# lukefleed/two-pass-lanczos

Hardware: AMD Instinct MI355X
Metric: Lanczos iterations/sec + SpMV GB/s (vs HBM roofline), 500k-arc KKT k=500 (higher is better)
Workload: dtype f64

## Files before the change

two-pass-lanczos_amd/csrc/tpl_device.h:

```cpp
#pragma once
#include <stdint.h>

namespace tpl {

constexpr int kTPB = 256;
#ifndef TPL_CHUNK_ROWS
#define TPL_CHUNK_ROWS 512
#endif
constexpr int kChunkRows = TPL_CHUNK_ROWS;
constexpr int kRowsPerThread = kChunkRows / kTPB;
#ifndef TPL_ELEM_ROWS
#define TPL_ELEM_ROWS 2048
#endif
constexpr int kElemRows = TPL_ELEM_ROWS;
constexpr int kElemMinBlocks = 192;
constexpr int kShortRowMax = 32;
#ifndef TPL_MAX_SLICES
#define TPL_MAX_SLICES 8
#endif
constexpr int kSlices = TPL_MAX_SLICES;
#ifndef TPL_SLOT_STRIDE
#define TPL_SLOT_STRIDE TPL_MAX_SLICES
#endif
constexpr int kSlotStride = TPL_SLOT_STRIDE;
// ... 15 lines not shown
constexpr int kWinLoads = kWinMax / 256;
constexpr int kFusedWidth = 4;
constexpr int kFusedHubMax = kTPB;
constexpr int kFusedLongMax = 2048;
constexpr int kBinMax = 7936;
constexpr int kCntStride = 16;
constexpr double kBreakdownTol = 2.220446049250313080847263336181640625e-13;

inline int p2_flush(int j, int last) {
  return (j % 3 == 0 || j == last) ? j - ((j - 1) / 3) * 3 : 0;
}

struct BinSeg {
  int32_t start, ri, row, pad;
};

struct CsrDev {
  const int32_t* srows;
  const void* s_col;
  const int32_t* s_cbase;
  const void* s_val;
  const int32_t* c_base;
  const int32_t* c_width;
  const void* b_col;
  const int32_t* b_cbase;
  const void* b_val;
  const BinSeg* b_seg;
  const int32_t* b_hdr;
  double* P;
  unsigned int* Pcnt;
// ... 128 lines not shown
```

two-pass-lanczos_amd/csrc/tpl_k_p2_fused.hip:

```cpp
#include "tpl_klaunch.h"

namespace tpl {

constexpr int kHubAhead = 8;

struct FusedP2Args {
  const int32_t* h_row;
  const int32_t* h_ent;
  const double* h_val;
  int32_t n_open, n_hub;
  double* ycache;
  const double* rec;
  const int32_t* flags;
  const double* v1;
  double* x;
  int64_t n;
  int32_t n_long;
  int32_t steps;
  const void* s_col;
  const void* s_val;
  const int32_t* s_cbase;
  const int32_t* c_base;
  const int32_t* c_width;
  int32_t n_short, n_chunks, s_width, val_i8, s_col16;
};

// ... 9 lines not shown
  return {readlane_f64(cv, 0), readlane_f64(cv, 1), readlane_f64(cv, 2), readlane_f64(cv, 3)};
}
__device__ __forceinline__ void fused_step_r(double s, const StepRec& r, double& vc, double& vp,
                                             double& xv) {
  double w = s - r.beta_sub * vp;
  w = w - r.alpha * vc;
  const double vn = w * r.invb;
  xv = xv + r.ycoef * vn;
  vp = vc;
  vc = vn;
}
__device__ __forceinline__ void fused_step(double s, double cv, double& vc, double& vp, double& xv) {
  fused_step_r(s, rec_fields(cv), vc, vp, xv);
}

constexpr uint32_t kLaneOff = 0x80000000u;
__device__ __forceinline__ void st_cache_row(double* row, int nl, uint32_t off, double v) {
  typedef uint32_t u32x2 __attribute__((ext_vector_type(2)));
  const __amdgpu_buffer_rsrc_t r = __builtin_amdgcn_make_buffer_rsrc(row, 0, nl * 8, 0x00020000);
  u32x2 d;
  d.x = (uint32_t)__double2loint(v);
  d.y = (uint32_t)__double2hiint(v);
  __builtin_amdgcn_raw_buffer_store_b64(d, r, off, 0, 0);
}

enum HubMode { kHubLong, kHubLds, kHubWave };
constexpr int kWave = 64;
template <HubMode MODE>
__device__ __forceinline__ void hub_chain(const FusedP2Args& a, double (*vh)[kTPB], int last,
                                          int lc, bool writes, bool open,
                                          const int (&ent)[kFusedWidth],
                                          const double (&av)[kFusedWidth], double& vc, double& vp,
                                          double& xv) {
  const int t = threadIdx.x;
  const int nl = a.n_long;
  double yb[kHubAhead], cb[kHubAhead];
#pragma unroll
  for (int u = 0; u < kHubAhead; ++u) {
    const int jj = clampi(1 + u, last);
    yb[u] = a.ycache[(size_t)(jj - 1) * nl + lc];
    cb[u] = a.rec[8 * (size_t)jj + (t & 7)];
  }
  const uint32_t soff = writes ? (uint32_t)lc * 8u : kLaneOff;
  auto step = [&](int j, double s, double cv) {
    st_cache_row(a.ycache + (size_t)(j - 1) * nl, nl, soff, vc);
    if (MODE == kHubLds) {
      double* vb = vh[j & 1];
      vb[t] = vc;
      __syncthreads();
      if (open) {
        s = 0.0;
#pragma unroll
        for (int k = 0; k < kFusedWidth; ++k) {
          const double prod = av[k] * vb[ent[k] < 0 ? 0 : ent[k]];
          s = s + (ent[k] >= 0 ? prod : -0.0);
        }
      }
    }
    if (MODE == kHubWave) {
      double so = 0.0;
#pragma unroll
      for (int k = 0; k < kFusedWidth; ++k) {
        const double prod = av[k] * __shfl(vc, ent[k] < 0 ? 0 : ent[k], kWave);
        so = so + (ent[k] >= 0 ? prod : -0.0);
      }
      s = open ? so : s;
    }
    fused_step(s, cv, vc, vp, xv);
  };
  const int nblk = last / kHubAhead;
  int j0 = 1;
  if (nblk > 0) __builtin_amdgcn_s_waitcnt(0x0F70);
  for (int b = 0; b < nblk; ++b, j0 += kHubAhead) {
#pragma unroll
    for (int u = 0; u < kHubAhead; ++u) {
      const int j = j0 + u;
      step(j, yb[u], cb[u]);
      __builtin_amdgcn_sched_barrier(0);
      const int jn = clampi(j + kHubAhead, last);
      yb[u] = a.ycache[(size_t)(jn - 1) * nl + lc];
      cb[u] = a.rec[8 * (size_t)jn + (t & 7)];
    }
  }
  const int rem = last - nblk * kHubAhead;
#pragma unroll
  for (int u = 0; u < kHubAhead - 1; ++u) {
    if (u >= rem) break;
    step(j0 + u, yb[u], cb[u]);
  }
}

__global__ __launch_bounds__(kTPB) void k_p2_hub(FusedP2Args a) {
  __shared__ double vh[2][kTPB];
  const int steps = fused_steps(a);
  if (steps < 2) return;
  const int last = steps - 1;
  const int t = threadIdx.x;
  const int nl = a.n_long;
  const int64_t first_long = a.n - nl;
  const int n_lb = (nl + kTPB - 1) / kTPB;
  const bool hub = (int)blockIdx.x >= n_lb;
  bool live, open = false;
  int lc;
  int64_t row;
  int ent[kFusedWidth];
  double av[kFusedWidth];
#pragma unroll
  for (int k = 0; k < kFusedWidth; ++k) {
    ent[k] = -1;
    av[k] = 0.0;
  }
  if (hub) {
    live = t < a.n_hub;
    open = t < a.n_open;
    row = a.h_row[clampi(t, a.n_hub - 1)];
    lc = open ? 0 : clampi((int)(row - first_long), nl - 1);
    if (open) {
#pragma unroll
      for (int k = 0; k < kFusedWidth; ++k) {
        ent[k] = a.h_ent[t * kFusedWidth + k];
        av[k] = a.h_val[t * kFusedWidth + k];
      }
    }
  } else {
    const int l = blockIdx.x * kTPB + t;
    lc = clampi(l, nl - 1);
    row = first_long + lc;
    live = l < nl;
    for (int h = a.n_open; h < a.n_hub; ++h) live = live && a.h_row[h] != (int32_t)row;
  }
  double vc = a.v1[row], vp = 0.0, xv = a.x[row];
  if (hub && a.n_hub <= kWave) {
    if (t >= kWave) return;
    hub_chain<kHubWave>(a, vh, last, lc, live && !open, open, ent, av, vc, vp, xv);
  } else if (hub) {
    hub_chain<kHubLds>(a, vh, last, lc, live && !open, open, ent, av, vc, vp, xv);
  } else {
    hub_chain<kHubLong>(a, vh, last, lc, live, false, ent, av, vc, vp, xv);
  }
  if (live) st_out(a.x + row, xv);
}

__device__ __forceinline__ int fused_col(const FusedP2Args& a, int e, int cbase) {
  if (a.s_col16) {
    const int off = reinterpret_cast<const uint16_t*>(a.s_col)[e];
    return off == 0xFFFF ? -1 : cbase + off;
  }
  return reinterpret_cast<const int32_t*>(a.s_col)[e];
}
__device__ __forceinline__ double fused_val(const FusedP2Args& a, int e) {
  if (a.val_i8) return (double)reinterpret_cast<const int8_t*>(a.s_val)[e];
  return reinterpret_cast<const double*>(a.s_val)[e];
}

constexpr int kRowsGroup = 4;
constexpr int kRowsThreads = kTPB * kRowsGroup;
constexpr int kRowsDepth = 2;

template <int W, int NL>
__global__ __launch_bounds__(kRowsThreads) void k_p2_rows(FusedP2Args a) {
  extern __shared__ double lds[];
  constexpr int NLC = (NL + kRowsGroup - 1) / kRowsGroup;
  constexpr int D = kRowsDepth;
  const int steps = fused_steps(a);
  if (steps < 2) return;
  const int last = steps - 1;
  const int tw = threadIdx.x;
  const int t = tw % kTPB;
  const int chunk_w = blockIdx.x * kRowsGroup + tw / kTPB;
  const bool have = chunk_w < a.n_chunks;
  const int chunk = have ? chunk_w : a.n_chunks - 1;
  const int nl = a.n_long;
  const int first_long = (int)(a.n - nl);
  const int wc = a.s_width > 0 ? a.s_width : a.c_width[chunk];
  const int base = a.s_width > 0 ? chunk * kChunkRows * a.s_width : a.c_base[chunk];
  const bool packed = a.s_width > 0 && packed_chunk_width(a.s_width);
  const int cbase = a.s_col16 ? a.s_cbase[chunk] : 0;
  int row[kRowsPerThread];
  bool live[kRowsPerThread];
  int li[kRowsPerThread][W];
  double av[kRowsPerThread][W];
// ... 20 lines not shown
      li[q][k] = idx;
    }
    vc[q] = a.v1[row[q]];
    vp[q] = 0.0;
    xv[q] = a.x[row[q]];
  }
  double st[D][NLC], cvr[D];
#pragma unroll
  for (int d = 0; d < D; ++d) {
    const int jj = clampi(1 + d, last);
#pragma unroll
    for (int u = 0; u < NLC; ++u)
      st[d][u] = a.ycache[(size_t)(jj - 1) * nl + clampi(tw + u * kRowsThreads, nl - 1)];
    cvr[d] = a.rec[8 * (size_t)jj + (tw & 7)];
  }
  auto step = [&](int j, int d, auto refill) {
    double* vb = lds + (j & 1) * nl;
#pragma unroll
    for (int u = 0; u < NLC; ++u)
      if (u < NLC - 1 || tw + u * kRowsThreads < nl) vb[tw + u * kRowsThreads] = st[d][u];
    const StepRec r = rec_fields(cvr[d]);
    if (decltype(refill)::value) {
      __builtin_amdgcn_sched_barrier(0);
      const int jn = clampi(j + D, last);
#pragma unroll
      for (int u = 0; u < NLC; ++u)
        st[d][u] = a.ycache[(size_t)(jn - 1) * nl + clampi(tw + u * kRowsThreads, nl - 1)];
      cvr[d] = a.rec[8 * (size_t)jn + (tw & 7)];
    }
    __syncthreads();
#pragma unroll
    for (int q = 0; q < kRowsPerThread; ++q) {
      double s = 0.0;
#pragma unroll
      for (int k = 0; k < W; ++k) {
        const double g = vb[li[q][k] < 0 ? 0 : li[q][k]];
        const double prod = av[q][k] * (li[q][k] == -2 ? vc[q] : g);
        s = s + (li[q][k] != -1 ? prod : -0.0);
      }
      fused_step_r(s, r, vc[q], vp[q], xv[q]);
    }
  };
  const int nblk = last / D;
  int j0 = 1;
  if (nblk > 0) __builtin_amdgcn_s_waitcnt(0x0F70);
  for (int b = 0; b < nblk; ++b, j0 += D) {
#pragma unroll
    for (int d = 0; d < D; ++d) step(j0 + d, d, std::true_type{});
  }
  const int rem = last - nblk * D;
#pragma unroll
  for (int d = 0; d < D - 1; ++d) {
    if (d >= rem) break;
    step(j0 + d, d, std::false_type{});
  }
#pragma unroll
  for (int q = 0; q < kRowsPerThread; ++q)
    if (live[q]) st_out(a.x + row[q], xv[q]);
}

namespace launch {

static FusedP2Args fused_args(const CsrDev& A, const DevState& S, const double* ycache,
                              const double* v1, double* x, int steps) {
  FusedP2Args a{};
  a.ycache = const_cast<double*>(ycache);
  a.rec = S.p2c;
  a.flags = S.flags;
  a.v1 = v1;
  a.x = x;
  a.n = A.n;
  a.n_long = A.n_long;
  a.steps = steps;
  a.s_col = A.s_col;
  a.s_val = A.s_val;
  a.s_cbase = A.s_cbase;
  a.c_base = A.c_base;
  a.c_width = A.c_width;
  a.n_short = A.n_short;
  a.n_chunks = A.n_chunks;
  a.s_width = A.s_width;
  a.val_i8 = A.val_i8;
  a.s_col16 = A.s_col16;
  return a;
}

hipError_t p2_fused_hub(const CsrDev& A, const DevState& S, const FusedP2Dev& H, double* ycache,
                        const double* v1, double* x, int steps, hipStream_t s) {
  if (A.n_long <= 0 || !A.s_identity || H.n_hub > kFusedHubMax || H.n_open > H.n_hub)
    return hipErrorInvalidConfiguration;
  FusedP2Args a = fused_args(A, S, ycache, v1, x, steps);
  a.h_row = H.h_row;
  a.h_ent = H.h_ent;
  a.h_val = H.h_val;
  a.n_open = H.n_open;
  a.n_hub = H.n_hub;
  const int grid = (A.n_long + kTPB - 1) / kTPB + (H.n_hub > 0 ? 1 : 0);
  hipLaunchKernelGGL(k_p2_hub, dim3(grid), dim3(kTPB), 0, s, a);
  return hipGetLastError();
}

template <int W, int... NLs>
static bool rows_nl(int nloads, const FusedP2Args& a, int grid, size_t lds, hipStream_t s,
                    std::integer_sequence<int, NLs...>) {
  auto one = [&](auto NL) {
    if (nloads != decltype(NL)::value + 1) return false;
    hipLaunchKernelGGL((k_p2_rows<W, decltype(NL)::value + 1>), dim3(grid), dim3(kRowsThreads),
                       lds, s, a);
    return true;
  };
  return (one(std::integral_constant<int, NLs>{}) || ...);
}

hipError_t p2_fused_rows(const CsrDev& A, const DevState& S, const double* ycache,
                         const double* v1, double* x, int steps, hipStream_t s) {
  if (A.n_long <= 0 || A.n_long > kFusedLongMax || !A.s_identity)
    return hipErrorInvalidConfiguration;
  if (A.n_chunks <= 0) return hipSuccess;
  const FusedP2Args a = fused_args(A, S, ycache, v1, x, steps);
  const size_t lds = 2 * (size_t)A.n_long * sizeof(double);
  const int nloads = (A.n_long + kTPB - 1) / kTPB;
  constexpr auto nls = std::make_integer_sequence<int, kFusedLongMax / kTPB>{};
  const int w = A.s_width > 0 ? A.s_width : kFusedWidth;
  const int grid = (A.n_chunks + kRowsGroup - 1) / kRowsGroup;
  bool ok = false;
  switch (w) {
    case 1: ok = rows_nl<1>(nloads, a, grid, lds, s, nls); break;
    case 2: ok = rows_nl<2>(nloads, a, grid, lds, s, nls); break;
    case 3: ok = rows_nl<3>(nloads, a, grid, lds, s, nls); break;
    case 4: ok = rows_nl<4>(nloads, a, grid, lds, s, nls); break;
    default: break;
  }
  return ok ? hipGetLastError() : hipErrorInvalidConfiguration;
}

}
}
```

two-pass-lanczos_amd/csrc/tpl_kcommon.h:

```cpp
#pragma once
#include <hip/hip_runtime.h>
#include "tpl_device.h"
#include "tpl_lab.h"

namespace tpl {

template <int kCtrl>
__device__ __forceinline__ double dpp_f64(double v) {
  const long long b = __double_as_longlong(v);
  const int lo = __builtin_amdgcn_update_dpp(0, (int)b, kCtrl, 0xF, 0xF, false);
  const int hi = __builtin_amdgcn_update_dpp(0, (int)(b >> 32), kCtrl, 0xF, 0xF, false);
  return __longlong_as_double(((long long)hi << 32) | (unsigned int)lo);
}
__device__ __forceinline__ double swz_xor16_f64(double v) {
  const long long b = __double_as_longlong(v);
  const int lo = __builtin_amdgcn_ds_swizzle((int)b, 0x401F);
  const int hi = __builtin_amdgcn_ds_swizzle((int)(b >> 32), 0x401F);
  return __longlong_as_double(((long long)hi << 32) | (unsigned int)lo);
}
__device__ __forceinline__ double readlane_f64(double v, int l) {
  const long long b = __double_as_longlong(v);
  const int lo = __builtin_amdgcn_readlane((int)b, l);
  const int hi = __builtin_amdgcn_readlane((int)(b >> 32), l);
  return __longlong_as_double(((long long)hi << 32) | (unsigned int)lo);
// ... 84 lines not shown

struct PreNone {};
__device__ __forceinline__ bool defer_long_y(const CsrDev& A, int ri, double y) {
  if (!A.long_defer) return false;
  A.ypart[ri] = y;
  return true;
}
struct EpiSpmv {
  double* y;
  __device__ __forceinline__ PreNone pre(int) const { return {}; }
  __device__ __forceinline__ double apply(int i, double s, const PreNone&, double&) const {
    st_out(y + i, s);
    return s;
  }
  __device__ __forceinline__ void long_alpha(int, double) const {}
  __device__ __forceinline__ bool long_y(const CsrDev& A, int ri, double y) const {
    return defer_long_y(A, ri, y);
  }
};

struct Pre1 {
  double rc, rp;
};
struct EpiPass1 {
  const double* r_cur;
  const double* r_prev;
  bool has_prev;
  double invN_cur, invN_prev, beta_sub;
  double* W;
  double* Vcol;
  double* Pa_long;
  __device__ __forceinline__ Pre1 pre(int i) const { return Pre1{r_cur[i], r_prev[i]}; }
  __device__ __forceinline__ void long_alpha(int r, double acc) const { st_out(Pa_long + r, acc); }
  __device__ __forceinline__ bool long_y(const CsrDev& A, int ri, double y) const {
    double* yp = A.ypart;
    if (yp) st_out(yp + ri, y);
    return A.long_defer != 0;
  }
  __device__ __forceinline__ double apply(int i, double s, const Pre1& p, double& acc) const {
    const double v = p.rc * invN_cur;
    const double vp = has_prev ? p.rp * invN_prev : 0.0;
    const double w = s - beta_sub * vp;
    st_out(W + i, w);
    if (Vcol) Vcol[i] = v;
    acc = fma(v, w, acc);
    return v;
  }
};

struct Pre2R {
  double vc, vp, x, cv;
};
// ... 30 lines not shown
    const double vp = has_prev ? p.vp : 0.0;
    double w = s - beta_sub * vp;
    w = w - alpha * p.vc;
    const double vn = w * invb;
    st_out(v_next + i, vn);
    if (nflush) {
      double xv = p.x;
      if (nflush >= 3) xv = xv + readlane_f64(p.cv, 5) * p.vp;
      if (nflush >= 2) xv = xv + readlane_f64(p.cv, 4) * p.vc;
      st_out(x + i, xv + ycoef * vn);
    }
    if (Vcol) Vcol[i] = vn;
    return vn;
  }
  __device__ __forceinline__ void long_alpha(int, double) const {}
  __device__ __forceinline__ bool long_y(const CsrDev& A, int ri, double y) const {
    return defer_long_y(A, ri, y);
  }
};

__device__ __forceinline__ void pin_layout_args(const CsrDev& A) {
  asm volatile("" ::"s"(A.s_col), "s"(A.s_val), "s"(A.s_cbase), "s"(A.b_col), "s"(A.b_val),
               "s"(A.b_seg), "s"(A.b_hdr), "s"(A.b_cbase));
  asm volatile("" ::"s"(A.n_short), "s"(A.n_slice_blocks), "s"(A.n_slices), "s"(A.bin_cap),
               "s"(A.s_identity), "s"(A.n_chunks));
}

__device__ __forceinline__ void keep_pre(PreNone&) {}
__device__ __forceinline__ void keep_pre(Pre1& p) { keep(p.rc); keep(p.rp); }
__device__ __forceinline__ void keep_pre(Pre2R& p) { keep(p.vc); keep(p.vp); keep(p.x); keep(p.cv); }

// ... 322 lines not shown
        acc = group8_sum(acc);
        if (g8 == 0 && valid) psum[j] = acc;
      }
    }
  }
  TPL_MARK(7);
  TPL_MARK(8);
  __syncthreads();
  TPL_MARK(3);
  keep_pre(pre);
  if (sg.ri < 0) return;
  const double p = psum[t];
  const int ns = A.n_slices;
  if (ns == 1 || sg.pad == 0) {
    const double y = 0.0 + p;
    if (epi.long_y(A, sg.ri, y)) return;
    double acc = 0.0;
    epi.apply(sg.row, y, pre, acc);
    epi.long_alpha(sg.ri, acc);
    return;
  }
  unsigned long long* slots = reinterpret_cast<unsigned long long*>(A.P + (size_t)sg.ri * kSlotStride);
  __hip_atomic_store(slots + s, (unsigned long long)__double_as_longlong(p), __ATOMIC_RELAXED,
                     __HIP_MEMORY_SCOPE_AGENT);
  asm volatile("s_waitcnt vmcnt(0)" ::: "memory");
  TPL_MARK(4);
  const unsigned int arrived = __builtin_amdgcn_atomic_inc32(
      A.Pcnt + (size_t)sg.ri * kCntStride, (unsigned)sg.pad, __ATOMIC_RELAXED, "agent");
  asm volatile("" ::: "memory");
  if (arrived != (unsigned)sg.pad) return;
  static_assert(kSlices == 8, "four slot pairs");
// ... 7 lines not shown
  asm volatile(
      "global_load_dwordx4 %0, %4, off sc1\n\t"
      "global_load_dwordx4 %1, %5, off sc1\n\t"
      "global_load_dwordx4 %2, %6, off sc1\n\t"
      "global_load_dwordx4 %3, %7, off sc1\n\t"
      "s_waitcnt vmcnt(0)"
      : "=&v"(r0), "=&v"(r1), "=&v"(r2), "=&v"(r3)
      : "v"(p0), "v"(p1), "v"(p2), "v"(p3)
      : "memory");
  v[0] = r0.x; v[1] = r0.y; v[2] = r1.x; v[3] = r1.y;
  v[4] = r2.x; v[5] = r2.y; v[6] = r3.x; v[7] = r3.y;
  double y = 0.0;
#pragma unroll
  for (int k = 0; k < kSlices; ++k)
    if (k < ns) y = y + __longlong_as_double((long long)v[k]);
  if (epi.long_y(A, sg.ri, y)) return;
  double acc = 0.0;
  epi.apply(sg.row, y, pre, acc);
  epi.long_alpha(sg.ri, acc);
}

__device__ __forceinline__ int rb_first(int G2, int x) { return (x * G2 + 7) >> 3; }
__device__ __forceinline__ int elem_block(int G2, int i) {
  const int x = i & 7, q = i >> 3;
  const int rb = rb_first(G2, x) + q;
  return rb < rb_first(G2, x + 1) ? rb : -1;
}
__device__ __forceinline__ int elem_block(const CsrDev& A, int i) { return elem_block(A.G2, i); }
__device__ __forceinline__ int chunk_of_block(const CsrDev& A, int i) {
  const int cpe = (int)(A.E / kChunkRows);
  const int x = (i + A.n_slice_blocks) & 7, q = i >> 3;
// ... 162 lines not shown
```

two-pass-lanczos_amd/csrc/tpl_launch.h:

```cpp
#pragma once
#include <hip/hip_runtime.h>

#include "tpl_device.h"

namespace tpl {
struct BatchDev;
namespace launch {
hipError_t spmv(const CsrDev& A, const double* x, double* y, hipStream_t s);
hipError_t p1_init(const CsrDev& A, const DevState& S, const double* b, hipStream_t s);
hipError_t p1_spmv(const CsrDev& A, const DevState& S, const double* xsrc, const double* r_cur,
                   const double* r_prev, double* W, double* Vcol, int j, hipStream_t s,
                   unsigned long long* stamp = nullptr);
hipError_t p1_axpy(const CsrDev& A, const DevState& S, const double* W, const double* r_cur,
                   double* r_next, int j, int k, int elim, hipStream_t s,
                   unsigned long long* stamp = nullptr);
hipError_t p1_axpy_tol(const CsrDev& A, const DevState& S, const double* W, const double* r_cur,
                       double* r_next, int j, int k, double* tr, hipStream_t s);
hipError_t p1_tol_fin(const DevState& S, double* tr, hipStream_t s);
struct ShiftTol {
  const double* tol;
  const double* sig;
  double* lu;
  double* st;
  double* res;
// ... 20 lines not shown
                               double* Y, int32_t* back, int scale, hipStream_t s);
hipError_t p2_init(int64_t n, const DevState& S, const double* b, double* v1, double* x,
                   double* Vcol, int dyn, hipStream_t s);
hipError_t p2_spmv(const CsrDev& A, const DevState& S, const double* xsrc, const double* v_cur,
                   const double* v_prev, double* v_next, double* x, double* Vcol, int j,
                   int nflush, hipStream_t s);
hipError_t p2_cached(const CsrDev& A, const DevState& S, const double* xsrc, const double* v_cur,
                     const double* v_prev, double* v_next, double* x, double* Vcol,
                     const double* ycache, const int32_t* lrow, int j, int nflush,
                     hipStream_t s);
struct FusedP2Dev {
  const int32_t *h_row, *h_ent;
  const double* h_val;
  int32_t n_open, n_hub;
};
hipError_t p2_fused_hub(const CsrDev& A, const DevState& S, const FusedP2Dev& H, double* ycache,
                        const double* v1, double* x, int steps, hipStream_t s);
hipError_t p2_fused_rows(const CsrDev& A, const DevState& S, const double* ycache,
                         const double* v1, double* x, int steps, hipStream_t s);
hipError_t bp2_cached(int nb, const CsrDev& A, const BatchDev& B, const double* v_cur,
                      const double* v_prev, double* v_next, double* x, const double* ycrow,
                      const int32_t* lrow, int j, hipStream_t s);
hipError_t p2_coefs(const DevState& S, int k, int dyn, hipStream_t s);
hipError_t gemv_recon(int64_t n, int steps, const DevState& S, const double* V, double* x,
                      hipStream_t s);
hipError_t p2_minit(const CsrDev& A, const DevState& S, const double* Y, int ldy, const double* b,
                    double* v1, double* X, int64_t ldx, int m, hipStream_t s);
hipError_t p2_xacc(const CsrDev& A, const double* Y, int ldy, int j, int nflush, const double* vp,
                   const double* vc, const double* vn, double* X, int64_t ldx, int m,
                   hipStream_t s);
int long_epi_blocks(const CsrDev& A);
hipError_t long_epi_p1(const CsrDev& A, const DevState& S, const double* yall, int R,
                       const double* r_cur, const double* r_prev, double* W, double* Vcol,
                       double* Pa_long, int j, hipStream_t s);
// ... 14 lines not shown
```

two-pass-lanczos_amd/csrc/tpl_op.h:

```cpp
#pragma once
#include <hip/hip_runtime.h>

#include <algorithm>
#include <cstdlib>
#include <cstring>
#include <functional>
#include <map>
#include <memory>
#include <new>
#include <string>
#include <vector>

#include "tpl_batch.h"
#include "tpl_device.h"
#include "tpl_internal.h"
#include "tpl_launch.h"
#include "tpl_layout.h"
#include "tpl_partition.h"

typedef struct ncclComm* ncclComm_t;

namespace tpl {

#define HIPCHK(expr)                                                                        \
// ... 227 lines not shown

struct HostDecomp {
  int32_t flags[kFlagBytes / 4];
  double b_norm;
  const double* alphas;
  const double* betas;
  size_t steps;
};

bool use_graphs();
GraphExec capture_graph(tpl_op_s* op, const std::function<void()>& enqueue);
void enqueue_reorth(tpl_op_s* op, int j, int mode);
void enqueue_p1_prologue(tpl_op_s* op);
void enqueue_p1_step(tpl_op_s* op, int j, int k, double* Vcol, bool elim = false,
                     unsigned long long* st1 = nullptr, unsigned long long* st2 = nullptr,
                     double* ycrow = nullptr);
void launch_p2_step(tpl_op_s* op, const CsrDev& A, int j, int t, int nflush, double* Vcol);
void launch_bp2_step(tpl_op_s* op, const CsrDev& A, int nb, int j);
void enqueue_pass2(tpl_op_s* op, size_t steps, double* Vout);
void enqueue_ftk_only(tpl_op_s* op, size_t k, int f, int scale);
void run_pass_one(tpl_op_s* op, const double* b, size_t k, int mem, bool storeV, int reorth,
                  bool elim = false);
void run_pass2(tpl_op_s* op, size_t steps);
void run_pass2_multi(tpl_op_s* op, size_t steps, size_t m);
void run_pass2_multi_cut(tpl_op_s* op, size_t steps, size_t m);
void run_pass1_batch(tpl_op_s* op, size_t k, int nb);
void run_pass2_batch(tpl_op_s* op, size_t kmax, int nb);
void run_pass2_batch_multi(tpl_op_s* op, const size_t* steps, int nb, size_t m);
void run_two_pass_dev(tpl_op_s* op, size_t k, int f);
void run_two_pass_inv_tol(tpl_op_s* op, size_t kmax);
void run_two_pass_shifted_inv_tol(tpl_op_s* op, size_t kmax, const launch::ShiftTol& t);
// ... 4 lines not shown
```

two-pass-lanczos_amd/csrc/tpl_passes.cpp:

```cpp
#include "tpl_op.h"

namespace tpl {

namespace {
enum GraphKind {
  kGPass1 = 0,
  kGPass2 = 16, kGPass2Steps,
  kGTwoPassDev,
  kGDevFtk,
  kGPass2Dyn,
  kGPass2Multi,
  kGPass1Batch,
  kGPass2Batch,
  kGPass2BatchMulti,
  kGTwoPassInvTol,
  kGPass2MultiCut,
  kGTwoPassShiftedInvTol,
  kGLongCache = 64,
  kGFusedP2 = 128,
};
enum P1Props { kP1Basis = 1, kP1Elim = 2, kP1Stamped = 4, kP1Cache = 8 };

inline double* cache_row(const tpl_op_s* op, int j) {
  return (size_t)j <= long_cache_steps(op)
             ? op->st.d_ycache + (size_t)(j - 1) * op->lay.lrows.size() : nullptr;
}
inline int graph_cache_kind(const tpl_op_s* op) {
  return long_cache_steps(op) ? kGLongCache | (fused_p2(op) ? kGFusedP2 : 0) : 0;
}
inline double* batch_cache_row(const tpl_op_s* op, int j, int nb) {
  return (size_t)j <= batch_cache_steps(op)
             ? op->bat.d_ycache + (size_t)(j - 1) * op->lay.lrows.size() * (size_t)nb : nullptr;
}
inline int batch_graph_cache_kind(const tpl_op_s* op) {
  return batch_cache_steps(op) ? kGLongCache : 0;
}

inline double* r_of(const tpl_op_s* op, int j) { return j == 1 ? op->b : op->R[j % 3]; }
inline double* rG_of(const tpl_op_s* op, int j) { return j == 1 ? op->bG : op->RG[j % 3]; }

struct P2Rot {
  double *G, *cur, *prev, *next;
};
// ... 24 lines not shown
    HIPCHK(launch::reorth_reduce(cols, P, G2, h, sk, op->stream));
    double* pn = pass == 1 ? op->st.S.Pb : (mode == 2 ? Pb1 : nullptr);
    HIPCHK(launch::reorth_update(op->part.n, cols, op->d_V, r, h, pn, G2, E, sk, op->stream));
    if (mode == 2 && pass == 0)
      HIPCHK(launch::reorth_decide(op->st.S, Pb1, G2, skip, rec, op->stream));
  }
}

void enqueue_p1_prologue(tpl_op_s* op) {
  const CsrDev A = csr_dev(op);
  HIPCHK(launch::p1_init(A, op->st.S, op->b, op->stream));
  if (op->dist) enqueue_p1_exchange_norm(op, A, op->bG);
}

void enqueue_p1_step(tpl_op_s* op, int j, int k, double* Vcol, bool elim, unsigned long long* st1,
                     unsigned long long* st2, double* ycrow) {
  CsrDev A = csr_dev(op, true);
  if (ycrow && !op->dist) A.ypart = ycrow;
  HIPCHK(launch::p1_spmv(A, op->st.S, rG_of(op, j), r_of(op, j), j >= 2 ? r_of(op, j - 1) : nullptr,
                         op->W, Vcol, j, op->stream, st1));
  if (op->dist) enqueue_p1_exchange_a(op, A);
  if (op->part.hybrid)
    HIPCHK(launch::long_epi_p1(A, op->st.S, op->d_yall, op->dist->nranks, r_of(op, j),
                               j >= 2 ? r_of(op, j - 1) : nullptr, op->W, Vcol,
                               op->d_rsum + op->dist->nranks, j, op->stream));
  HIPCHK(launch::p1_axpy(A, op->st.S, op->W, r_of(op, j), op->R[(j + 1) % 3], j, k,
                         elim ? 1 : 0, op->stream, st2));
  if (op->dist && j < k) enqueue_p1_exchange_norm(op, A, op->RG[(j + 1) % 3]);
}

static int stamp_first(size_t k) {
  return k >= (size_t)kStampSteps + 3 ? (int)(k - kStampSteps) / 2 + 1 : 0;
}

static void enqueue_pass1(tpl_op_s* op, size_t k, int props, int reorth = 0) {
  enqueue_p1_prologue(op);
  const int js = props & kP1Stamped ? stamp_first(k) : 0;
  for (int j = 1; j <= (int)k; ++j) {
    double* Vcol = props & kP1Basis ? op->d_V + (size_t)(j - 1) * op->part.n : nullptr;
    const int i = j - js;
    unsigned long long* st1 = js && i >= 0 && i <= kStampSteps ? op->d_stamps + 2 * i : nullptr;
    unsigned long long* st2 = js && i >= 0 && i < kStampSteps ? op->d_stamps + 2 * i + 1 : nullptr;
    enqueue_p1_step(op, j, (int)k, Vcol, (props & kP1Elim) != 0, st1, st2,
                    props & kP1Cache ? cache_row(op, j) : nullptr);
    if (reorth && j < (int)k) enqueue_reorth(op, j, reorth);
  }
}

static void enqueue_pass2_init(tpl_op_s* op, size_t steps, double* Vout) {
  HIPCHK(launch::p2_init(op->part.n, op->st.S, op->b, op->V2[1], op->x, Vout, 0, op->stream));
  HIPCHK(launch::p2_coefs(op->st.S, (int)steps, 0, op->stream));
  if (op->dist && !op->part.hybrid) {
    halo_pack(op, op->V2G[1]);
    gather_vec(op, op->V2G[1]);
  }
}

void launch_p2_step(tpl_op_s* op, const CsrDev& A, int j, int t, int nflush, double* Vcol) {
  const P2Rot v = p2_rot(op, t);
// ... 16 lines not shown
      const P2Rot v = p2_rot(op, j);
      enqueue_p2_exchange(op, j);
      HIPCHK(launch::long_epi_p2(A, op->st.S, op->d_yall, op->dist->nranks, v.cur,
                                 j >= 2 ? v.prev : nullptr, v.next, op->x, Vcol, j, nflush,
                                 op->stream));
    } else if (op->dist && j + 1 < (int)steps) {
      enqueue_p2_exchange(op, j);
    }
  }
}
static void enqueue_pass2_fused(tpl_op_s* op, size_t steps) {
  const CsrDev A = csr_dev(op);
  const FusedP2& f = op->lay.fp2;
  const launch::FusedP2Dev H{op->bufs.d_hrow, op->bufs.d_hent, op->bufs.d_hval, (int32_t)f.n_open,
                             (int32_t)f.n_hub};
  HIPCHK(launch::p2_fused_hub(A, op->st.S, H, op->st.d_ycache, op->V2[1], op->x, (int)steps,
                              op->stream));
  HIPCHK(launch::p2_fused_rows(A, op->st.S, op->st.d_ycache, op->V2[1], op->x, (int)steps,
                               op->stream));
}
void enqueue_pass2(tpl_op_s* op, size_t steps, double* Vout) {
  enqueue_pass2_init(op, steps, Vout);
  enqueue_pass2_steps(op, steps, Vout);
}

void enqueue_ftk_only(tpl_op_s* op, size_t k, int f, int scale) {
  if (f == kDevExp)
    HIPCHK(launch::ftk_exp(op->st.S, (int)k, scale, op->stream));
  else
    HIPCHK(launch::ftk_inv(op->st.S, (int)k, scale, op->stream));
}
static void enqueue_ftk_dev(tpl_op_s* op, size_t k, int f) {
  enqueue_ftk_only(op, k, f, 1);
  HIPCHK(launch::p2_init(op->part.n, op->st.S, op->b, op->V2[1], op->x, nullptr, 1, op->stream));
// ... 39 lines not shown
    return;
  }
  auto it = op->graphs.find({kind, key});
  if (it == op->graphs.end()) {
    GraphExec ge = capture_graph(op, [&] { enqueue(); });
    if (!ge) {
      enqueue();
      return;
    }
    it = op->graphs.emplace(std::make_pair(kind, key), std::move(ge)).first;
  }
  HIPCHK(hipGraphLaunch(it->second.get(), op->stream));
}

static void run_pass1_graph(tpl_op_s* op, size_t k, int props) {
  if (long_cache_steps(op)) props |= kP1Cache;
  run_graph(op, kGPass1 + props, k, [&] { enqueue_pass1(op, k, props); });
}

void run_pass2(tpl_op_s* op, size_t steps) {
  op->last_long_cache = steps >= 2 && long_cache_steps(op) > 0;
  const bool fused = fused_p2(op);
  op->last_fused_p2 = steps >= 2 && fused;
  auto enqueue_steps = [&] {
    if (fused) enqueue_pass2_fused(op, steps);
    else enqueue_pass2_steps(op, steps, nullptr);
  };
  if (!op->timing) {
    run_graph(op, kGPass2 + graph_cache_kind(op), steps, [&] {
      enqueue_pass2_init(op, steps, nullptr);
      enqueue_steps();
// ... 59 lines not shown
void run_pass2_multi_cut(tpl_op_s* op, size_t steps, size_t m) {
  check_multi_cut(op, steps, m);
  op->last_long_cache = steps >= 2 && long_cache_steps(op) > 0;
  run_graph(op, kGPass2MultiCut + graph_cache_kind(op), steps * (TPL_MULTI_MAX + 1) + m,
            [&] { enqueue_pass2_multi_cut(op, steps, m, false); });
}

void run_two_pass_shifted_inv_tol(tpl_op_s* op, size_t kmax, const launch::ShiftTol& t) {
  const size_t m = (size_t)t.m;
  check_multi_cut(op, kmax, m);
  const int ck = graph_cache_kind(op);
  op->last_long_cache = kmax >= 2 && ck != 0;
  run_graph(op, kGTwoPassShiftedInvTol + ck, kmax * (TPL_MULTI_MAX + 1) + m, [&] {
    enqueue_p1_prologue(op);
    for (int j = 1; j <= (int)kmax; ++j) {
      CsrDev A = csr_dev(op, true);
      if (double* ycrow = ck ? cache_row(op, j) : nullptr) A.ypart = ycrow;
      HIPCHK(launch::p1_spmv(A, op->st.S, rG_of(op, j), r_of(op, j),
                             j >= 2 ? r_of(op, j - 1) : nullptr, op->W, nullptr, j, op->stream,
                             nullptr));
      HIPCHK(launch::p1_axpy_stol(A, op->st.S, op->W, r_of(op, j), op->R[(j + 1) % 3], j,
                                  (int)kmax, t, op->stream));
    }
    HIPCHK(launch::p1_stol_fin(op->st.S, t, op->stream));
    HIPCHK(launch::ftk_inv_shifts(op->st.S, (int)kmax, t, op->d_Y, (int)op->ycap,
                                  op->d_col_steps, 1, op->stream));
    enqueue_pass2_multi_cut(op, kmax, m, true);
  });
}

static void enqueue_pass1_batch(tpl_op_s* op, size_t k, int nb) {
  const CsrDev A = csr_dev(op);
// ... 97 lines not shown
  d.betas = d.alphas + kc;
  d.steps = (size_t)d.flags[2];
  return d;
}

void run_two_pass_dev(tpl_op_s* op, size_t k, int f) {
  const size_t key = 2 * k + (size_t)f;
  const int elim = f == kDevInv ? kP1Elim : 0;
  const int ck = graph_cache_kind(op);
  op->last_long_cache = k >= 2 && ck != 0;
  const bool fused = fused_p2(op);
  op->last_fused_p2 = k >= 2 && fused;
  if (!op->timing) {
    op->p1_samples = 0;
    run_graph(op, kGTwoPassDev + ck, key, [&] {
      enqueue_pass1(op, k, elim | (ck ? kP1Cache : 0));
      enqueue_ftk_dev(op, k, f);
      if (fused) {
        enqueue_pass2_fused(op, 0);
      } else {
        enqueue_pass2_dyn_steps(op, k);
        enqueue_pass2_tail(op);
      }
    });
    return;
  }
  HIPCHK(hipEventRecord(op->tev[0], op->stream));
  const bool stamped = !op->dist && stamp_first(k) > 0;
  if (stamped && !op->d_stamps) {
    dev_alloc(op, &op->d_stamps, 32 * sizeof(unsigned long long));
    HIPCHK(hipMemset(op->d_stamps, 0, 32 * sizeof(unsigned long long)));
// ... 8 lines not shown
    else enqueue_pass2_dyn_steps(op, k);
  });
  HIPCHK(hipEventRecord(op->tev[3], op->stream));
  if (!fused) enqueue_pass2_tail(op);
  op->p2_launches = (int64_t)k - 1;
}

void run_two_pass_inv_tol(tpl_op_s* op, size_t kmax) {
  const int ck = graph_cache_kind(op);
  op->last_long_cache = kmax >= 2 && ck != 0;
  const bool fused = fused_p2(op);
  op->last_fused_p2 = kmax >= 2 && fused;
  run_graph(op, kGTwoPassInvTol + ck, kmax, [&] {
    enqueue_p1_prologue(op);
    for (int j = 1; j <= (int)kmax; ++j) {
      CsrDev A = csr_dev(op, true);
      if (double* ycrow = ck ? cache_row(op, j) : nullptr) A.ypart = ycrow;
      HIPCHK(launch::p1_spmv(A, op->st.S, rG_of(op, j), r_of(op, j),
                             j >= 2 ? r_of(op, j - 1) : nullptr, op->W, nullptr, j, op->stream,
                             nullptr));
      HIPCHK(launch::p1_axpy_tol(A, op->st.S, op->W, r_of(op, j), op->R[(j + 1) % 3], j,
                                 (int)kmax, op->d_tol, op->stream));
    }
    HIPCHK(launch::p1_tol_fin(op->st.S, op->d_tol, op->stream));
    enqueue_ftk_dev(op, kmax, kDevInv);
    if (fused) {
      enqueue_pass2_fused(op, 0);
    } else {
      enqueue_pass2_dyn_steps(op, kmax);
      enqueue_pass2_tail(op);
    }
  });
// ... 19 lines not shown
```

Baseline: 92330.

## Cache long-row Lanczos vectors in pass one and merge fused pass-two kernels

When the fused pass two is in use, pass one now stores the normalized Lanczos vector entries for long rows into the cache (KeepV mode) instead of their partial SpMV sums. Pass two can then rebuild x for long rows as a plain dot product over cached vectors and coefficients, with no recurrence to replay. The long-row and small-hub work move into side blocks of the rows kernel, so one launch does what two did, and the rows kernel now stages D steps of LDS at once to cut barriers. The cost is twice the LDS per workgroup and a more complex grid split.

Result: no change. 93240 (median of 6 runs) (+1.0%).

```diff
diff --git a/two-pass-lanczos_amd/csrc/tpl_device.h b/two-pass-lanczos_amd/csrc/tpl_device.h
--- a/two-pass-lanczos_amd/csrc/tpl_device.h
+++ b/two-pass-lanczos_amd/csrc/tpl_device.h
@@ -53,6 +53,9 @@
 struct BinSeg {
   int32_t start, ri, row, pad;
 };
+
+constexpr int kLongDefer = 1;
+constexpr int kLongKeepV = 2;
 
 struct CsrDev {
   const int32_t* srows;
diff --git a/two-pass-lanczos_amd/csrc/tpl_k_p2_fused.hip b/two-pass-lanczos_amd/csrc/tpl_k_p2_fused.hip
--- a/two-pass-lanczos_amd/csrc/tpl_k_p2_fused.hip
+++ b/two-pass-lanczos_amd/csrc/tpl_k_p2_fused.hip
@@ -9,7 +9,7 @@
   const int32_t* h_ent;
   const double* h_val;
   int32_t n_open, n_hub;
-  double* ycache;
+  const double* ycache;
   const double* rec;
   const int32_t* flags;
   const double* v1;
@@ -49,22 +49,11 @@
   fused_step_r(s, rec_fields(cv), vc, vp, xv);
 }
 
-constexpr uint32_t kLaneOff = 0x80000000u;
-__device__ __forceinline__ void st_cache_row(double* row, int nl, uint32_t off, double v) {
-  typedef uint32_t u32x2 __attribute__((ext_vector_type(2)));
-  const __amdgpu_buffer_rsrc_t r = __builtin_amdgcn_make_buffer_rsrc(row, 0, nl * 8, 0x00020000);
-  u32x2 d;
-  d.x = (uint32_t)__double2loint(v);
-  d.y = (uint32_t)__double2hiint(v);
-  __builtin_amdgcn_raw_buffer_store_b64(d, r, off, 0, 0);
-}
-
-enum HubMode { kHubLong, kHubLds, kHubWave };
+enum HubMode { kHubLds, kHubWave };
 constexpr int kWave = 64;
 template <HubMode MODE>
 __device__ __forceinline__ void hub_chain(const FusedP2Args& a, double (*vh)[kTPB], int last,
-                                          int lc, bool writes, bool open,
-                                          const int (&ent)[kFusedWidth],
+                                          int lc, bool open, const int (&ent)[kFusedWidth],
                                           const double (&av)[kFusedWidth], double& vc, double& vp,
                                           double& xv) {
   const int t = threadIdx.x;
@@ -76,30 +65,25 @@
     yb[u] = a.ycache[(size_t)(jj - 1) * nl + lc];
     cb[u] = a.rec[8 * (size_t)jj + (t & 7)];
   }
-  const uint32_t soff = writes ? (uint32_t)lc * 8u : kLaneOff;
-  auto step = [&](int j, double s, double cv) {
-    st_cache_row(a.ycache + (size_t)(j - 1) * nl, nl, soff, vc);
+  auto step = [&](int j, double vj, double cv) {
+    vc = open ? vc : vj;
+    double s = 0.0;
     if (MODE == kHubLds) {
       double* vb = vh[j & 1];
       vb[t] = vc;
       __syncthreads();
-      if (open) {
-        s = 0.0;
-#pragma unroll
-        for (int k = 0; k < kFusedWidth; ++k) {
-          const double prod = av[k] * vb[ent[k] < 0 ? 0 : ent[k]];
-          s = s + (ent[k] >= 0 ? prod : -0.0);
-        }
+#pragma unroll
+      for (int k = 0; k < kFusedWidth; ++k) {
+        const double prod = av[k] * vb[ent[k] < 0 ? 0 : ent[k]];
+        s = s + (ent[k] >= 0 ? prod : -0.0);
       }
     }
     if (MODE == kHubWave) {
-      double so = 0.0;
 #pragma unroll
       for (int k = 0; k < kFusedWidth; ++k) {
         const double prod = av[k] * __shfl(vc, ent[k] < 0 ? 0 : ent[k], kWave);
-        so = so + (ent[k] >= 0 ? prod : -0.0);
-      }
-      s = open ? so : s;
+        s = s + (ent[k] >= 0 ? prod : -0.0);
+      }
     }
     fused_step(s, cv, vc, vp, xv);
   };
@@ -125,55 +109,77 @@
   }
 }
 
+template <HubMode MODE>
+__device__ __forceinline__ void hub_block(const FusedP2Args& a, double (*vh)[kTPB], int last) {
+  const int t = threadIdx.x;
+  const int nl = a.n_long;
+  const bool open = t < a.n_open;
+  const int64_t row = a.h_row[clampi(t, a.n_hub - 1)];
+  const int lo = (int)(row - (a.n - nl));
+  const int lc = lo < 0 ? 0 : clampi(lo, nl - 1);
+  int ent[kFusedWidth];
+  double av[kFusedWidth];
+#pragma unroll
+  for (int k = 0; k < kFusedWidth; ++k) {
+    ent[k] = -1;
+    av[k] = 0.0;
+  }
+  if (open) {
+#pragma unroll
+    for (int k = 0; k < kFusedWidth; ++k) {
+      ent[k] = a.h_ent[t * kFusedWidth + k];
+      av[k] = a.h_val[t * kFusedWidth + k];
+    }
+  }
+  double vc = a.v1[row], vp = 0.0, xv = a.x[row];
+  hub_chain<MODE>(a, vh, last, lc, open, ent, av, vc, vp, xv);
+  if (open) st_out(a.x + row, xv);
+}
+
 __global__ __launch_bounds__(kTPB) void k_p2_hub(FusedP2Args a) {
   __shared__ double vh[2][kTPB];
   const int steps = fused_steps(a);
   if (steps < 2) return;
-  const int last = steps - 1;
-  const int t = threadIdx.x;
+  hub_block<kHubLds>(a, vh, steps - 1);
+}
+
+constexpr int kRowsGroup = 4;
+constexpr int kRowsThreads = kTPB * kRowsGroup;
+constexpr int kRowsDepth = 2;
+
+__device__ __forceinline__ void long_rows_x(const FusedP2Args& a, int last, int lb) {
   const int nl = a.n_long;
-  const int64_t first_long = a.n - nl;
-  const int n_lb = (nl + kTPB - 1) / kTPB;
-  const bool hub = (int)blockIdx.x >= n_lb;
-  bool live, open = false;
-  int lc;
-  int64_t row;
-  int ent[kFusedWidth];
-  double av[kFusedWidth];
-#pragma unroll
-  for (int k = 0; k < kFusedWidth; ++k) {
-    ent[k] = -1;
-    av[k] = 0.0;
-  }
-  if (hub) {
-    live = t < a.n_hub;
-    open = t < a.n_open;
-    row = a.h_row[clampi(t, a.n_hub - 1)];
-    lc = open ? 0 : clampi((int)(row - first_long), nl - 1);
-    if (open) {
-#pragma unroll
-      for (int k = 0; k < kFusedWidth; ++k) {
-        ent[k] = a.h_ent[t * kFusedWidth + k];
-        av[k] = a.h_val[t * kFusedWidth + k];
-      }
-    }
-  } else {
-    const int l = blockIdx.x * kTPB + t;
-    lc = clampi(l, nl - 1);
-    row = first_long + lc;
-    live = l < nl;
-    for (int h = a.n_open; h < a.n_hub; ++h) live = live && a.h_row[h] != (int32_t)row;
-  }
-  double vc = a.v1[row], vp = 0.0, xv = a.x[row];
-  if (hub && a.n_hub <= kWave) {
-    if (t >= kWave) return;
-    hub_chain<kHubWave>(a, vh, last, lc, live && !open, open, ent, av, vc, vp, xv);
-  } else if (hub) {
-    hub_chain<kHubLds>(a, vh, last, lc, live && !open, open, ent, av, vc, vp, xv);
-  } else {
-    hub_chain<kHubLong>(a, vh, last, lc, live, false, ent, av, vc, vp, xv);
-  }
-  if (live) st_out(a.x + row, xv);
+  const int l = lb * kRowsThreads + (int)threadIdx.x;
+  const int lc = clampi(l, nl - 1);
+  const int64_t row = a.n - nl + lc;
+  double xv = a.x[row];
+  double vb[kHubAhead], yb[kHubAhead];
+#pragma unroll
+  for (int u = 0; u < kHubAhead; ++u) {
+    const int jj = clampi(1 + u, last);
+    vb[u] = a.ycache[(size_t)jj * nl + lc];
+    yb[u] = a.rec[8 * (size_t)jj + 3];
+  }
+  const int nblk = last / kHubAhead;
+  int j0 = 1;
+  if (nblk > 0) __builtin_amdgcn_s_waitcnt(0x0F70);
+  for (int b = 0; b < nblk; ++b, j0 += kHubAhead) {
+#pragma unroll
+    for (int u = 0; u < kHubAhead; ++u) {
+      xv = xv + yb[u] * vb[u];
+      __builtin_amdgcn_sched_barrier(0);
+      const int jn = clampi(j0 + u + kHubAhead, last);
+      vb[u] = a.ycache[(size_t)jn * nl + lc];
+      yb[u] = a.rec[8 * (size_t)jn + 3];
+    }
+  }
+  const int rem = last - nblk * kHubAhead;
+#pragma unroll
+  for (int u = 0; u < kHubAhead - 1; ++u) {
+    if (u >= rem) break;
+    xv = xv + yb[u] * vb[u];
+  }
+  if (l < nl) st_out(a.x + row, xv);
 }
 
 __device__ __forceinline__ int fused_col(const FusedP2Args& a, int e, int cbase) {
@@ -187,10 +193,6 @@
   if (a.val_i8) return (double)reinterpret_cast<const int8_t*>(a.s_val)[e];
   return reinterpret_cast<const double*>(a.s_val)[e];
 }
-
-constexpr int kRowsGroup = 4;
-constexpr int kRowsThreads = kTPB * kRowsGroup;
-constexpr int kRowsDepth = 2;
 
 template <int W, int NL>
 __global__ __launch_bounds__(kRowsThreads) void k_p2_rows(FusedP2Args a) {
@@ -200,6 +202,16 @@
   const int steps = fused_steps(a);
   if (steps < 2) return;
   const int last = steps - 1;
+  const int side = (int)blockIdx.x - (a.n_chunks + kRowsGroup - 1) / kRowsGroup;
+  if (side >= 0) {
+    const int n_lb = (a.n_long + kRowsThreads - 1) / kRowsThreads;
+    if (side < n_lb) {
+      long_rows_x(a, last, side);
+    } else if (threadIdx.x < kWave) {
+      hub_block<kHubWave>(a, nullptr, last);
+    }
+    return;
+  }
   const int tw = threadIdx.x;
   const int t = tw % kTPB;
   const int chunk_w = blockIdx.x * kRowsGroup + tw / kTPB;
@@ -250,46 +262,51 @@
       st[d][u] = a.ycache[(size_t)(jj - 1) * nl + clampi(tw + u * kRowsThreads, nl - 1)];
     cvr[d] = a.rec[8 * (size_t)jj + (tw & 7)];
   }
-  auto step = [&](int j, int d, auto refill) {
-    double* vb = lds + (j & 1) * nl;
-#pragma unroll
-    for (int u = 0; u < NLC; ++u)
-      if (u < NLC - 1 || tw + u * kRowsThreads < nl) vb[tw + u * kRowsThreads] = st[d][u];
-    const StepRec r = rec_fields(cvr[d]);
+  auto block = [&](int b, int j0, int nd, auto refill) {
+    double* vb0 = lds + (b & 1) * (D * nl);
+    StepRec r[D];
+#pragma unroll
+    for (int d = 0; d < D; ++d) {
+#pragma unroll
+      for (int u = 0; u < NLC; ++u)
+        if (u < NLC - 1 || tw + u * kRowsThreads < nl) vb0[d * nl + tw + u * kRowsThreads] = st[d][u];
+      r[d] = rec_fields(cvr[d]);
+    }
     if (decltype(refill)::value) {
       __builtin_amdgcn_sched_barrier(0);
-      const int jn = clampi(j + D, last);
-#pragma unroll
-      for (int u = 0; u < NLC; ++u)
-        st[d][u] = a.ycache[(size_t)(jn - 1) * nl + clampi(tw + u * kRowsThreads, nl - 1)];
-      cvr[d] = a.rec[8 * (size_t)jn + (tw & 7)];
+#pragma unroll
+      for (int d = 0; d < D; ++d) {
+        const int jn = clampi(j0 + d + D, last);
+#pragma unroll
+        for (int u = 0; u < NLC; ++u)
+          st[d][u] = a.ycache[(size_t)(jn - 1) * nl + clampi(tw + u * kRowsThreads, nl - 1)];
+        cvr[d] = a.rec[8 * (size_t)jn + (tw & 7)];
+      }
     }
     __syncthreads();
 #pragma unroll
-    for (int q = 0; q < kRowsPerThread; ++q) {
-      double s = 0.0;
-#pragma unroll
-      for (int k = 0; k < W; ++k) {
-        const double g = vb[li[q][k] < 0 ? 0 : li[q][k]];
-        const double prod = av[q][k] * (li[q][k] == -2 ? vc[q] : g);
-        s = s + (li[q][k] != -1 ? prod : -0.0);
-      }
-      fused_step_r(s, r, vc[q], vp[q], xv[q]);
+    for (int d = 0; d < D; ++d) {
+      if (d >= nd) break;
+      const double* vb = vb0 + d * nl;
+#pragma unroll
+      for (int q = 0; q < kRowsPerThread; ++q) {
+        double s = 0.0;
+#pragma unroll
+        for (int k = 0; k < W; ++k) {
+          const double g = vb[li[q][k] < 0 ? 0 : li[q][k]];
+          const double prod = av[q][k] * (li[q][k] == -2 ? vc[q] : g);
+          s = s + (li[q][k] != -1 ? prod : -0.0);
+        }
+        fused_step_r(s, r[d], vc[q], vp[q], xv[q]);
+      }
     }
   };
   const int nblk = last / D;
   int j0 = 1;
   if (nblk > 0) __builtin_amdgcn_s_waitcnt(0x0F70);
-  for (int b = 0; b < nblk; ++b, j0 += D) {
-#pragma unroll
-    for (int d = 0; d < D; ++d) step(j0 + d, d, std::true_type{});
-  }
+  for (int b = 0; b < nblk; ++b, j0 += D) block(b, j0, D, std::true_type{});
   const int rem = last - nblk * D;
-#pragma unroll
-  for (int d = 0; d < D - 1; ++d) {
-    if (d >= rem) break;
-    step(j0 + d, d, std::false_type{});
-  }
+  if (rem > 0) block(nblk, j0, rem, std::false_type{});
 #pragma unroll
   for (int q = 0; q < kRowsPerThread; ++q)
     if (live[q]) st_out(a.x + row[q], xv[q]);
@@ -297,10 +314,15 @@
 
 namespace launch {
 
-static FusedP2Args fused_args(const CsrDev& A, const DevState& S, const double* ycache,
-                              const double* v1, double* x, int steps) {
+static FusedP2Args fused_args(const CsrDev& A, const DevState& S, const FusedP2Dev& H,
+                              const double* ycache, const double* v1, double* x, int steps) {
   FusedP2Args a{};
-  a.ycache = const_cast<double*>(ycache);
+  a.h_row = H.h_row;
+  a.h_ent = H.h_ent;
+  a.h_val = H.h_val;
+  a.n_open = H.n_open;
+  a.n_hub = H.n_hub;
+  a.ycache = ycache;
   a.rec = S.p2c;
   a.flags = S.flags;
   a.v1 = v1;
@@ -321,21 +343,6 @@
   return a;
 }
 
-hipError_t p2_fused_hub(const CsrDev& A, const DevState& S, const FusedP2Dev& H, double* ycache,
-                        const double* v1, double* x, int steps, hipStream_t s) {
-  if (A.n_long <= 0 || !A.s_identity || H.n_hub > kFusedHubMax || H.n_open > H.n_hub)
-    return hipErrorInvalidConfiguration;
-  FusedP2Args a = fused_args(A, S, ycache, v1, x, steps);
-  a.h_row = H.h_row;
-  a.h_ent = H.h_ent;
-  a.h_val = H.h_val;
-  a.n_open = H.n_open;
-  a.n_hub = H.n_hub;
-  const int grid = (A.n_long + kTPB - 1) / kTPB + (H.n_hub > 0 ? 1 : 0);
-  hipLaunchKernelGGL(k_p2_hub, dim3(grid), dim3(kTPB), 0, s, a);
-  return hipGetLastError();
-}
-
 template <int W, int... NLs>
 static bool rows_nl(int nloads, const FusedP2Args& a, int grid, size_t lds, hipStream_t s,
                     std::integer_sequence<int, NLs...>) {
@@ -348,17 +355,25 @@
   return (one(std::integral_constant<int, NLs>{}) || ...);
 }
 
-hipError_t p2_fused_rows(const CsrDev& A, const DevState& S, const double* ycache,
-                         const double* v1, double* x, int steps, hipStream_t s) {
-  if (A.n_long <= 0 || A.n_long > kFusedLongMax || !A.s_identity)
+hipError_t p2_fused(const CsrDev& A, const DevState& S, const FusedP2Dev& H, const double* ycache,
+                    const double* v1, double* x, int steps, hipStream_t s) {
+  if (A.n_long <= 0 || A.n_long > kFusedLongMax || !A.s_identity || H.n_hub < 0 ||
+      H.n_hub > kFusedHubMax || H.n_open < 0 || H.n_open > H.n_hub)
     return hipErrorInvalidConfiguration;
-  if (A.n_chunks <= 0) return hipSuccess;
-  const FusedP2Args a = fused_args(A, S, ycache, v1, x, steps);
-  const size_t lds = 2 * (size_t)A.n_long * sizeof(double);
+  const FusedP2Args a = fused_args(A, S, H, ycache, v1, x, steps);
+  if (H.n_hub > kWave) {
+    hipLaunchKernelGGL(k_p2_hub, dim3(1), dim3(kTPB), 0, s, a);
+    if (const hipError_t e = hipGetLastError()) return e;
+  }
+  const size_t lds = 2 * kRowsDepth * (size_t)A.n_long * sizeof(double);
+  static_assert(2 * kRowsDepth * kFusedLongMax * sizeof(double) <= 64 * 1024, "one workgroup's LDS");
   const int nloads = (A.n_long + kTPB - 1) / kTPB;
   constexpr auto nls = std::make_integer_sequence<int, kFusedLongMax / kTPB>{};
   const int w = A.s_width > 0 ? A.s_width : kFusedWidth;
-  const int grid = (A.n_chunks + kRowsGroup - 1) / kRowsGroup;
+  const int n_chunks = A.n_chunks > 0 ? A.n_chunks : 0;
+  const int grid = (n_chunks + kRowsGroup - 1) / kRowsGroup +
+                   (A.n_long + kRowsThreads - 1) / kRowsThreads +
+                   (H.n_hub > 0 && H.n_hub <= kWave ? 1 : 0);
   bool ok = false;
   switch (w) {
     case 1: ok = rows_nl<1>(nloads, a, grid, lds, s, nls); break;
diff --git a/two-pass-lanczos_amd/csrc/tpl_kcommon.h b/two-pass-lanczos_amd/csrc/tpl_kcommon.h
--- a/two-pass-lanczos_amd/csrc/tpl_kcommon.h
+++ b/two-pass-lanczos_amd/csrc/tpl_kcommon.h
@@ -122,7 +122,8 @@
     return s;
   }
   __device__ __forceinline__ void long_alpha(int, double) const {}
-  __device__ __forceinline__ bool long_y(const CsrDev& A, int ri, double y) const {
+  template <class Pre>
+  __device__ __forceinline__ bool long_y(const CsrDev& A, int ri, double y, const Pre&) const {
     return defer_long_y(A, ri, y);
   }
 };
@@ -140,10 +141,11 @@
   double* Pa_long;
   __device__ __forceinline__ Pre1 pre(int i) const { return Pre1{r_cur[i], r_prev[i]}; }
   __device__ __forceinline__ void long_alpha(int r, double acc) const { st_out(Pa_long + r, acc); }
-  __device__ __forceinline__ bool long_y(const CsrDev& A, int ri, double y) const {
+  __device__ __forceinline__ bool long_y(const CsrDev& A, int ri, double y, const Pre1& p) const {
     double* yp = A.ypart;
-    if (yp) st_out(yp + ri, y);
-    return A.long_defer != 0;
+    const int mode = A.long_defer;
+    if (yp) st_out(yp + ri, mode == kLongKeepV ? p.rc * invN_cur : y);
+    return mode == kLongDefer;
   }
   __device__ __forceinline__ double apply(int i, double s, const Pre1& p, double& acc) const {
     const double v = p.rc * invN_cur;
@@ -204,7 +206,8 @@
     return vn;
   }
   __device__ __forceinline__ void long_alpha(int, double) const {}
-  __device__ __forceinline__ bool long_y(const CsrDev& A, int ri, double y) const {
+  template <class Pre>
+  __device__ __forceinline__ bool long_y(const CsrDev& A, int ri, double y, const Pre&) const {
     return defer_long_y(A, ri, y);
   }
 };
@@ -557,7 +560,7 @@
   const int ns = A.n_slices;
   if (ns == 1 || sg.pad == 0) {
     const double y = 0.0 + p;
-    if (epi.long_y(A, sg.ri, y)) return;
+    if (epi.long_y(A, sg.ri, y, pre)) return;
     double acc = 0.0;
     epi.apply(sg.row, y, pre, acc);
     epi.long_alpha(sg.ri, acc);
@@ -595,7 +598,7 @@
 #pragma unroll
   for (int k = 0; k < kSlices; ++k)
     if (k < ns) y = y + __longlong_as_double((long long)v[k]);
-  if (epi.long_y(A, sg.ri, y)) return;
+  if (epi.long_y(A, sg.ri, y, pre)) return;
   double acc = 0.0;
   epi.apply(sg.row, y, pre, acc);
   epi.long_alpha(sg.ri, acc);
diff --git a/two-pass-lanczos_amd/csrc/tpl_launch.h b/two-pass-lanczos_amd/csrc/tpl_launch.h
--- a/two-pass-lanczos_amd/csrc/tpl_launch.h
+++ b/two-pass-lanczos_amd/csrc/tpl_launch.h
@@ -58,10 +58,8 @@
   const double* h_val;
   int32_t n_open, n_hub;
 };
-hipError_t p2_fused_hub(const CsrDev& A, const DevState& S, const FusedP2Dev& H, double* ycache,
-                        const double* v1, double* x, int steps, hipStream_t s);
-hipError_t p2_fused_rows(const CsrDev& A, const DevState& S, const double* ycache,
-                         const double* v1, double* x, int steps, hipStream_t s);
+hipError_t p2_fused(const CsrDev& A, const DevState& S, const FusedP2Dev& H, const double* ycache,
+                    const double* v1, double* x, int steps, hipStream_t s);
 hipError_t bp2_cached(int nb, const CsrDev& A, const BatchDev& B, const double* v_cur,
                       const double* v_prev, double* v_next, double* x, const double* ycrow,
                       const int32_t* lrow, int j, hipStream_t s);
diff --git a/two-pass-lanczos_amd/csrc/tpl_op.h b/two-pass-lanczos_amd/csrc/tpl_op.h
--- a/two-pass-lanczos_amd/csrc/tpl_op.h
+++ b/two-pass-lanczos_amd/csrc/tpl_op.h
@@ -265,7 +265,7 @@
 void enqueue_p1_prologue(tpl_op_s* op);
 void enqueue_p1_step(tpl_op_s* op, int j, int k, double* Vcol, bool elim = false,
                      unsigned long long* st1 = nullptr, unsigned long long* st2 = nullptr,
-                     double* ycrow = nullptr);
+                     int cache = 0);
 void launch_p2_step(tpl_op_s* op, const CsrDev& A, int j, int t, int nflush, double* Vcol);
 void launch_bp2_step(tpl_op_s* op, const CsrDev& A, int nb, int j);
 void enqueue_pass2(tpl_op_s* op, size_t steps, double* Vout);
diff --git a/two-pass-lanczos_amd/csrc/tpl_passes.cpp b/two-pass-lanczos_amd/csrc/tpl_passes.cpp
--- a/two-pass-lanczos_amd/csrc/tpl_passes.cpp
+++ b/two-pass-lanczos_amd/csrc/tpl_passes.cpp
@@ -5,7 +5,7 @@
 namespace {
 enum GraphKind {
   kGPass1 = 0,
-  kGPass2 = 16, kGPass2Steps,
+  kGPass2 = 32, kGPass2Steps,
   kGTwoPassDev,
   kGDevFtk,
   kGPass2Dyn,
@@ -19,7 +19,7 @@
   kGLongCache = 64,
   kGFusedP2 = 128,
 };
-enum P1Props { kP1Basis = 1, kP1Elim = 2, kP1Stamped = 4, kP1Cache = 8 };
+enum P1Props { kP1Basis = 1, kP1Elim = 2, kP1Stamped = 4, kP1Cache = 8, kP1CacheV = 16 };
 
 inline double* cache_row(const tpl_op_s* op, int j) {
   return (size_t)j <= long_cache_steps(op)
@@ -27,6 +27,18 @@
 }
 inline int graph_cache_kind(const tpl_op_s* op) {
   return long_cache_steps(op) ? kGLongCache | (fused_p2(op) ? kGFusedP2 : 0) : 0;
+}
+inline int p1_cache_props(const tpl_op_s* op) {
+  return long_cache_steps(op) ? kP1Cache | (fused_p2(op) ? kP1CacheV : 0) : 0;
+}
+inline CsrDev p1_step_dev(const tpl_op_s* op, int j, int props) {
+  CsrDev A = csr_dev(op, true);
+  double* row = (props & kP1Cache) && !op->dist ? cache_row(op, j) : nullptr;
+  if (row) {
+    A.ypart = row;
+    if (props & kP1CacheV) A.long_defer = kLongKeepV;
+  }
+  return A;
 }
 inline double* batch_cache_row(const tpl_op_s* op, int j, int nb) {
   return (size_t)j <= batch_cache_steps(op)
@@ -81,9 +93,8 @@
 }
 
 void enqueue_p1_step(tpl_op_s* op, int j, int k, double* Vcol, bool elim, unsigned long long* st1,
-                     unsigned long long* st2, double* ycrow) {
-  CsrDev A = csr_dev(op, true);
-  if (ycrow && !op->dist) A.ypart = ycrow;
+                     unsigned long long* st2, int cache) {
+  const CsrDev A = p1_step_dev(op, j, cache);
   HIPCHK(launch::p1_spmv(A, op->st.S, rG_of(op, j), r_of(op, j), j >= 2 ? r_of(op, j - 1) : nullptr,
                          op->W, Vcol, j, op->stream, st1));
   if (op->dist) enqueue_p1_exchange_a(op, A);
@@ -109,7 +120,7 @@
     unsigned long long* st1 = js && i >= 0 && i <= kStampSteps ? op->d_stamps + 2 * i : nullptr;
     unsigned long long* st2 = js && i >= 0 && i < kStampSteps ? op->d_stamps + 2 * i + 1 : nullptr;
     enqueue_p1_step(op, j, (int)k, Vcol, (props & kP1Elim) != 0, st1, st2,
-                    props & kP1Cache ? cache_row(op, j) : nullptr);
+                    props & (kP1Cache | kP1CacheV));
     if (reorth && j < (int)k) enqueue_reorth(op, j, reorth);
   }
 }
@@ -156,10 +167,8 @@
   const FusedP2& f = op->lay.fp2;
   const launch::FusedP2Dev H{op->bufs.d_hrow, op->bufs.d_hent, op->bufs.d_hval, (int32_t)f.n_open,
                              (int32_t)f.n_hub};
-  HIPCHK(launch::p2_fused_hub(A, op->st.S, H, op->st.d_ycache, op->V2[1], op->x, (int)steps,
-                              op->stream));
-  HIPCHK(launch::p2_fused_rows(A, op->st.S, op->st.d_ycache, op->V2[1], op->x, (int)steps,
-                               op->stream));
+  HIPCHK(launch::p2_fused(A, op->st.S, H, op->st.d_ycache, op->V2[1], op->x, (int)steps,
+                          op->stream));
 }
 void enqueue_pass2(tpl_op_s* op, size_t steps, double* Vout) {
   enqueue_pass2_init(op, steps, Vout);
@@ -229,7 +238,7 @@
 }
 
 static void run_pass1_graph(tpl_op_s* op, size_t k, int props) {
-  if (long_cache_steps(op)) props |= kP1Cache;
+  props |= p1_cache_props(op);
   run_graph(op, kGPass1 + props, k, [&] { enqueue_pass1(op, k, props); });
 }
 
@@ -319,8 +328,7 @@
   run_graph(op, kGTwoPassShiftedInvTol + ck, kmax * (TPL_MULTI_MAX + 1) + m, [&] {
     enqueue_p1_prologue(op);
     for (int j = 1; j <= (int)kmax; ++j) {
-      CsrDev A = csr_dev(op, true);
-      if (double* ycrow = ck ? cache_row(op, j) : nullptr) A.ypart = ycrow;
+      const CsrDev A = p1_step_dev(op, j, p1_cache_props(op));
       HIPCHK(launch::p1_spmv(A, op->st.S, rG_of(op, j), r_of(op, j),
                              j >= 2 ? r_of(op, j - 1) : nullptr, op->W, nullptr, j, op->stream,
                              nullptr));
@@ -448,7 +456,7 @@
   if (!op->timing) {
     op->p1_samples = 0;
     run_graph(op, kGTwoPassDev + ck, key, [&] {
-      enqueue_pass1(op, k, elim | (ck ? kP1Cache : 0));
+      enqueue_pass1(op, k, elim | p1_cache_props(op));
       enqueue_ftk_dev(op, k, f);
       if (fused) {
         enqueue_pass2_fused(op, 0);
@@ -487,8 +495,7 @@
   run_graph(op, kGTwoPassInvTol + ck, kmax, [&] {
     enqueue_p1_prologue(op);
     for (int j = 1; j <= (int)kmax; ++j) {
-      CsrDev A = csr_dev(op, true);
-      if (double* ycrow = ck ? cache_row(op, j) : nullptr) A.ypart = ycrow;
+      const CsrDev A = p1_step_dev(op, j, p1_cache_props(op));
       HIPCHK(launch::p1_spmv(A, op->st.S, rG_of(op, j), r_of(op, j),
                              j >= 2 ? r_of(op, j - 1) : nullptr, op->W, nullptr, j, op->stream,
                              nullptr));
```
